# jinggqu/NextGen-UIA

Hardware: AMD Instinct MI355X
Metric: images/sec fwd+bwd BiomedCLIP+Mona bs=256 (higher is better)
Workload: dtype bf16

## Files before the change

### nextgen-uia_amd/csrc/mona.hip

```cpp
#include <stdlib.h>
#include <type_traits>
#include "uia_common.h"
#include "uia_kernels.h"

#include "mona_spatial.h"

namespace {
using namespace uia_mona;

constexpr int LN_MAXV = 4;

template <typename T>
__global__ __launch_bounds__(256) void mona_pre_fwd_kernel(int M, int D, const float* __restrict__ x, const float* __restrict__ nw,
                                                            const float* __restrict__ nb, const float* __restrict__ gamma,
                                                            const float* __restrict__ gammax, float eps, T* __restrict__ u) {
    const int row = blockIdx.x * 4 + (threadIdx.x >> 6), lane = threadIdx.x & 63;
    if (row >= M) return;
    const int nv = D >> 2;
    const float* xr = x + (size_t)row * D;
    f32x4 v[LN_MAXV];
    float s = 0.f;
#pragma unroll
    for (int k = 0; k < LN_MAXV; ++k) {
        const int c = lane + 64 * k;
// ... 514 lines not shown
        sdc = red[c * 50 + 49];
#pragma unroll
        for (int i = 0; i < 7; ++i)
#pragma unroll
            for (int j = 0; j < 7; ++j) {
                grad_out(wsrow, WS_C3W, p.g_conv3_w, c * 49 + i * 7 + j, w3 * dkm[i * 7 + j]);
                if (i >= 1 && i <= 5 && j >= 1 && j <= 5) grad_out(wsrow, WS_C2W, p.g_conv2_w, c * 25 + (i - 1) * 5 + (j - 1), w2 * dkm[i * 7 + j]);
                if (i >= 2 && i <= 4 && j >= 2 && j <= 4) grad_out(wsrow, WS_C1W, p.g_conv1_w, c * 9 + (i - 2) * 3 + (j - 2), w1 * dkm[i * 7 + j]);
            }
        grad_out(wsrow, WS_C1B, p.g_conv1_b, c, w1 * sdc);
        grad_out(wsrow, WS_C2B, p.g_conv2_b, c, w2 * sdc);
        grad_out(wsrow, WS_C3B, p.g_conv3_b, c, w3 * sdc);
    }
    float dpool_c = 0.f;
    if (has_noise) {
        __syncthreads();
        float r1 = wave_sum(dwm1), r2 = wave_sum(dwm2), r3 = wave_sum(dwm3);
        if (c == 0) { scr[SCR_RED + grp * 4] = r1; scr[SCR_RED + grp * 4 + 1] = r2; scr[SCR_RED + grp * 4 + 2] = r3; }
        __syncthreads();
        if (tid < 16) {
            float dwv[3], wv[3] = {w1, w2, w3}, dl[3];
            for (int k = 0; k < 3; ++k) {
                dwv[k] = 0.f;
                for (int q = 0; q < NGRP; ++q) dwv[k] += scr[SCR_RED + 4 * q + k];
            }
            const float dot = dwv[0] * wv[0] + dwv[1] * wv[1] + dwv[2] * wv[2];
            for (int k = 0; k < 3; ++k) dl[k] = wv[k] * (dwv[k] - dot);
            const float hid = scr[SCR_HID + tid], hpre = scr[SCR_HPRE + tid];
            float dh = 0.f;
            for (int k = 0; k < 3; ++k) {
                grad_out(wsrow, WS_NE3W, p.g_ne3_w, k * 16 + tid, dl[k] * hid);
                dh = fmaf(dl[k], p.ne3_w[k * 16 + tid], dh);
            }
            if (tid < 3) grad_out(wsrow, WS_NE3B, p.g_ne3_b, tid, dl[tid]);
            dh = hpre > 0.f ? dh : 0.f;
            scr[SCR_HPRE + tid] = dh;
            grad_out(wsrow, WS_NE1B, p.g_ne1_b, tid, dh);
        }
        __syncthreads();
        if (tid < 64) {
            float dp = 0.f;
            for (int j = 0; j < 16; ++j) dp = fmaf(scr[SCR_HPRE + j], p.ne1_w[j * 64 + tid], dp);
            scr[SCR_DPOOL + tid] = dp / hw;
        }
        for (int i = tid; i < 16 * 64; i += 512) grad_out(wsrow, WS_NE1W, p.g_ne1_w, i, scr[SCR_HPRE + (i >> 6)] * scr[SCR_POOL + (i & 63)]);
        __syncthreads();
        dpool_c = scr[SCR_DPOOL + c];
    }
    float dfc = 0.f;
    T* dt = (T*)p.dt;
    for (int px = p0; px < p1; ++px) {
        const int y = px / w, x = px - y * w;
        float acc = 0.f;
#pragma unroll
        for (int i = 0; i < 7; ++i) {
            const int yy = y - (i - 3);
            const bool vy = yy >= 0 && yy < h;
#pragma unroll
            for (int j = 0; j < 7; ++j) {
                const int xx = x - (j - 3);
                const bool ok = vy && xx >= 0 && xx < w;
                const float gv = gS[(ok ? 1 + yy * w + xx : 0) * BOTT + c];
                acc = fmaf(KM(i, j), ok ? gv : 0.f, acc);
            }
        }
        const float dxf = acc + dpool_c;
        dfc = fmaf(dxf, tS[(1 + px) * BOTT + c], dfc);
        dt[(tok0 + 1 + px) * BOTT + c] = from_f32<T>(fmaf(f, dxf, gS[(1 + px) * BOTT + c]));
    }
    if (grp == 0) dt[tok0 * BOTT + c] = from_f32<T>(gS[c]);
    if (has_freq) {
        __syncthreads();
        scr[SCR_PART + grp * 64 + c] = dfc;
        __syncthreads();
        if (tid < 64) {
            float a = 0.f;
#pragma unroll
            for (int q = 0; q < NGRP; ++q) a += scr[SCR_PART + q * 64 + tid];
            grad_out(wsrow, WS_FREQ, p.g_freq, tid, a);
        }
    }
}

template <int W, bool BWD>
__global__ __launch_bounds__(512) void mona_spatial_fast_kernel(const uia_mona_spatial_desc p) {
    typedef bf16_t T;
    extern __shared__ __attribute__((aligned(16))) char smem[];
    const int h = p.h, hw = h * W, ntok = hw + 1;
    float* tS = (float*)smem;
    float* cS = tS + ntok * BOTT;
    const int cs_floats = (hw * FLD > FAST_RED) ? hw * FLD : FAST_RED;
    float* gS = cS + cs_floats;
    float* scr = BWD ? gS + ((ntok * FLD > KW_FLOATS) ? ntok * FLD : KW_FLOATS) : cS + cs_floats;
    const int tid = threadIdx.x, lane = tid & 63, c = lane, grp = tid >> 6;
    const int li = lane & 15, g = lane >> 4;
    const int b = blockIdx.x;
    const bool has_freq = p.variant == UIA_MONA_FREQ_ENHANCED || p.variant == UIA_MONA_HYBRID;
    const bool has_noise = p.variant == UIA_MONA_NOISE_AWARE || p.variant == UIA_MONA_HYBRID;
    const int ppg = (hw + NGRP - 1) / NGRP;
    const size_t tok0 = (size_t)b * ntok;
    float* wsrow = (BWD && p.ws) ? p.ws + (size_t)b * WS_ROW : nullptr;

    float* wst = BWD ? gS : scr + SCR_SIZE;
    for (int i = tid; i < KW_FLOATS / 4; i += 512) {
        const float* src = i < 144 ? p.conv1_w + 4 * i : (i < 544 ? p.conv2_w + 4 * (i - 144) : p.conv3_w + 4 * (i - 544));
        *(f32x4*)(wst + 4 * i) = load4(src);
    }
    load_tokens((const T*)p.t + tok0 * BOTT, tS, ntok, tid);
    __syncthreads();
#if defined(MSB_STOP) && MSB_STOP == 0
    if (BWD && p.B > 0) return;
#endif
    const float f = has_freq ? p.freq[c] : 1.0f;
    float w1 = 1.f / 3.f, w2 = 1.f / 3.f, w3 = 1.f / 3.f;
    if (has_noise) {
        noise_forward(p, tS, f, hw, ppg, c, grp, tid, scr);
        w1 = scr[SCR_W]; w2 = scr[SCR_W + 1]; w3 = scr[SCR_W + 2];
    }
    float km[49];
    {
        float k1[9], k2[25], k3[49];
#pragma unroll
        for (int i = 0; i < 9; ++i) k1[i] = wst[c * 9 + i];
#pragma unroll
        for (int i = 0; i < 25; ++i) k2[i] = wst[576 + c * 25 + i];
#pragma unroll
        for (int i = 0; i < 49; ++i) k3[i] = wst[2176 + c * 49 + i];
#pragma unroll
        for (int i = 0; i < 7; ++i)
#pragma unroll
            for (int j = 0; j < 7; ++j) km[i * 7 + j] = KM(i, j);
    }
    const float b1 = p.conv1_b[c], b2 = p.conv2_b[c], b3 = p.conv3_b[c];
    const float bm = w1 * b1 + w2 * b2 + w3 * b3;
#if defined(MSB_STOP) && MSB_STOP == 1
    if (BWD && p.B > 0) return;
#endif
    for (int y = grp; y < h; y += NGRP) {
        float acc[W];
#pragma unroll
        for (int x = 0; x < W; ++x) acc[x] = 0.f;
        stencil_row<W, false>(tS + BOTT, BOTT, h, y, c, km, acc);
#pragma unroll
        for (int x = 0; x < W; ++x) cS[(y * W + x) * FLD + c] = fmaf(f, acc[x], bm) + tS[(1 + y * W + x) * BOTT + c];
    }
    __syncthreads();

#if defined(MSB_STOP) && MSB_STOP == 2
    if (BWD && p.B > 0) return;
#endif
    const float inv_keep = p.p_drop > 0.f ? 1.0f / (1.0f - p.p_drop) : 1.0f;
    const uint32_t thresh = p.p_drop > 0.f ? (uint32_t)fminf(p.p_drop * 4294967296.0f, 4294967295.0f) : 0u;
    auto keep_scale = [&](int tok, int ch) -> float {
        const size_t idx = (tok0 + tok) * BOTT + ch;
        if (p.keep_mask) return p.keep_mask[idx] ? inv_keep : 0.f;
        if (p.p_drop > 0.f) return dropout_keep(p.seed, (uint32_t)idx, thresh) ? inv_keep : 0.f;
        return 1.0f;
    };
    const int mtiles = (hw + 15) >> 4;
    {
        bf16x8 pw[4][2];
        float pb[4];
#pragma unroll
        for (int nt = 0; nt < 4; ++nt) {
#pragma unroll
            for (int kk = 0; kk < 2; ++kk) {
                const float* src = p.proj_w + (16 * nt + li) * 64 + 32 * kk + 8 * g;
                pw[nt][kk] = pack8(load4(src), load4(src + 4));
            }
            pb[nt] = p.proj_b[16 * nt + li];
        }
        for (int mt = grp; mt < mtiles; mt += NGRP) {
            int arow = 16 * mt + li;
            arow = arow < hw ? arow : hw - 1;
            bf16x8 af[2];
#pragma unroll
            for (int kk = 0; kk < 2; ++kk) {
                const float* src = cS + arow * FLD + 32 * kk + 8 * g;
                af[kk] = pack8(*(const f32x4*)src, *(const f32x4*)(src + 4));
            }
#pragma unroll
            for (int nt = 0; nt < 4; ++nt) {
                f32x4 acc = f32x4{0.f, 0.f, 0.f, 0.f};
                acc = __builtin_amdgcn_mfma_f32_16x16x32_bf16(af[0], pw[nt][0], acc, 0, 0, 0);
                acc = __builtin_amdgcn_mfma_f32_16x16x32_bf16(af[1], pw[nt][1], acc, 0, 0, 0);
                const int co = 16 * nt + li;
#pragma unroll
                for (int r = 0; r < 4; ++r) {
                    const int px = 16 * mt + 4 * g + r;
                    if (px < hw) {
                        const float z = cS[px * FLD + co] + acc[r] + pb[nt];
                        const float ks = keep_scale(1 + px, co);
                        if (!BWD) ((T*)p.d)[(tok0 + 1 + px) * BOTT + co] = (T)(gelu_erf(z) * ks);
                        else gS[(1 + px) * FLD + co] = to_f32(((const T*)p.dd)[(tok0 + 1 + px) * BOTT + co]) * ks * dgelu_erf(z);
                    }
                }
            }
        }
        if (grp == NGRP - 1) {
            const float z = tS[c], ks = keep_scale(0, c);
            if (!BWD) ((T*)p.d)[tok0 * BOTT + c] = (T)(gelu_erf(z) * ks);
            else gS[c] = to_f32(((const T*)p.dd)[tok0 * BOTT + c]) * ks * dgelu_erf(z);
        }
    }
    if (!BWD) return;

#if defined(MSB_STOP) && MSB_STOP == 3
    if (BWD && p.B > 0) return;
#endif
    __syncthreads();
    {
        const int mt = grp & 3, nt0 = 2 * (grp >> 2);
        f32x4 acc[2] = {f32x4{0.f, 0.f, 0.f, 0.f}, f32x4{0.f, 0.f, 0.f, 0.f}};
        const int ksteps = (hw + 31) >> 5;
        for (int ks = 0; ks < ksteps; ++ks) {
            bf16x8 a, al, bb[2], bl[2];
#pragma unroll
            for (int e = 0; e < 8; ++e) {
                const int px = 32 * ks + 8 * g + e;
                const int pc = px < hw ? px : hw - 1;
                const float av = px < hw ? gS[(1 + pc) * FLD + 16 * mt + li] : 0.f;
                const float b0 = cS[pc * FLD + 16 * nt0 + li], b1 = cS[pc * FLD + 16 * (nt0 + 1) + li];
                a[e] = (bf16_t)av;      al[e] = (bf16_t)(av - (float)a[e]);
                bb[0][e] = (bf16_t)b0;  bl[0][e] = (bf16_t)(b0 - (float)bb[0][e]);
                bb[1][e] = (bf16_t)b1;  bl[1][e] = (bf16_t)(b1 - (float)bb[1][e]);
            }
#pragma unroll
            for (int q = 0; q < 2; ++q) {
                acc[q] = __builtin_amdgcn_mfma_f32_16x16x32_bf16(al, bb[q], acc[q], 0, 0, 0);
                acc[q] = __builtin_amdgcn_mfma_f32_16x16x32_bf16(a, bl[q], acc[q], 0, 0, 0);
                acc[q] = __builtin_amdgcn_mfma_f32_16x16x32_bf16(a, bb[q], acc[q], 0, 0, 0);
            }
        }
#pragma unroll
        for (int q = 0; q < 2; ++q)
#pragma unroll
            for (int r = 0; r < 4; ++r) grad_out(wsrow, WS_PROJ_W, p.g_proj_w, (16 * mt + 4 * g + r) * 64 + 16 * (nt0 + q) + li, acc[q][r]);
        {
            float sb = 0.f;
            for (int px = grp; px < hw; px += NGRP) sb += gS[(1 + px) * FLD + c];
            scr[SCR_PART + grp * 64 + c] = sb;
        }
    }
    __syncthreads();
#if defined(MSB_STOP) && MSB_STOP == 4
    if (BWD && p.B > 0) return;
#endif
    {
        bf16x8 pt[4][2];
#pragma unroll
        for (int nt = 0; nt < 4; ++nt)
#pragma unroll
            for (int kk = 0; kk < 2; ++kk)
#pragma unroll
                for (int e = 0; e < 8; ++e) pt[nt][kk][e] = (bf16_t)p.proj_w[(32 * kk + 8 * g + e) * 64 + 16 * nt + li];
        for (int mt = grp; mt < mtiles; mt += NGRP) {
            int arow = 16 * mt + li;
            arow = arow < hw ? arow : hw - 1;
            bf16x8 af[2];
#pragma unroll
            for (int kk = 0; kk < 2; ++kk) {
                const float* src = gS + (1 + arow) * FLD + 32 * kk + 8 * g;
                af[kk] = pack8(*(const f32x4*)src, *(const f32x4*)(src + 4));
            }
            f32x4 acc[4];
#pragma unroll
            for (int nt = 0; nt < 4; ++nt) {
                acc[nt] = __builtin_amdgcn_mfma_f32_16x16x32_bf16(af[0], pt[nt][0], f32x4{0.f, 0.f, 0.f, 0.f}, 0, 0, 0);
                acc[nt] = __builtin_amdgcn_mfma_f32_16x16x32_bf16(af[1], pt[nt][1], acc[nt], 0, 0, 0);
            }
            __builtin_amdgcn_wave_barrier();
#pragma unroll
            for (int nt = 0; nt < 4; ++nt)
#pragma unroll
                for (int r = 0; r < 4; ++r) {
                    const int px = 16 * mt + 4 * g + r;
                    if (px < hw) gS[(1 + px) * FLD + 16 * nt + li] += acc[nt][r];
                }
        }
    }
    __syncthreads();
#if defined(MSB_STOP) && MSB_STOP == 5
    if (BWD && p.B > 0) return;
#endif
    float dkm[49];
#pragma unroll
    for (int i = 0; i < 49; ++i) dkm[i] = 0.f;
    float sdc = 0.f, dwm1 = 0.f, dwm2 = 0.f, dwm3 = 0.f;
    for (int y = grp; y < h; y += NGRP) {
        float dcr[W];
#pragma unroll
        for (int x = 0; x < W; ++x) { dcr[x] = gS[(1 + y * W + x) * FLD + c]; sdc += dcr[x]; }
#pragma unroll
        for (int i = 0; i < 7; ++i) {
            const int yy = y + i - 3;
            if (yy < 0 || yy >= h) continue;
            float row[W + 6];
#pragma unroll
            for (int x = 0; x < W + 6; ++x) row[x] = 0.f;
#pragma unroll
            for (int x = 0; x < W; ++x) row[3 + x] = tS[(1 + yy * W + x) * BOTT + c];
#pragma unroll
            for (int j = 0; j < 7; ++j) {
                float a = 0.f;
#pragma unroll
                for (int x = 0; x < W; ++x) a = fmaf(dcr[x], row[x + j], a);
                dkm[i * 7 + j] += a;
            }
        }
    }
    if (has_noise) {
        float s1 = 0.f, s2 = 0.f, s3 = 0.f;
#pragma unroll
        for (int i = 0; i < 7; ++i)
#pragma unroll
            for (int j = 0; j < 7; ++j) {
                s3 = fmaf(p.conv3_w[c * 49 + i * 7 + j], dkm[i * 7 + j], s3);
                if (i >= 1 && i <= 5 && j >= 1 && j <= 5) s2 = fmaf(p.conv2_w[c * 25 + (i - 1) * 5 + (j - 1)], dkm[i * 7 + j], s2);
                if (i >= 2 && i <= 4 && j >= 2 && j <= 4) s1 = fmaf(p.conv1_w[c * 9 + (i - 2) * 3 + (j - 2)], dkm[i * 7 + j], s1);
            }
        dwm1 = fmaf(f, s1, b1 * sdc);
        dwm2 = fmaf(f, s2, b2 * sdc);
        dwm3 = fmaf(f, s3, b3 * sdc);
    }
#if defined(MSB_STOP) && MSB_STOP == 6
    if (BWD && p.B > 0) return;
#endif
    float* red = cS;
    constexpr int RST = 51, RW = 64 * RST;
    if (grp >= 4) {
        float* dst = red + (grp - 4) * RW + c * RST;
#pragma unroll
        for (int i = 0; i < 49; ++i) dst[i] = dkm[i];
        dst[49] = sdc;
    }
    __syncthreads();
    if (grp < 4) {
        float* dst = red + grp * RW + c * RST;
#pragma unroll
        for (int i = 0; i < 49; ++i) dst[i] += dkm[i];
        dst[49] += sdc;
    }
    __syncthreads();
    auto red4 = [&](int ch, int k) { const float* r = red + ch * RST + k; return (r[0] + r[RW]) + (r[2 * RW] + r[3 * RW]); };
    for (int i = tid; i < 64 * 49; i += 512) {
        const int ch = i / 49, k = i - 49 * ch;
        grad_out(wsrow, WS_C3W, p.g_conv3_w, i, w3 * (has_freq ? p.freq[ch] : 1.0f) * red4(ch, k));
    }
    for (int i = tid; i < 64 * 25; i += 512) {
        const int ch = i / 25, k = i - 25 * ch, ki = k / 5, kj = k - 5 * ki;
        grad_out(wsrow, WS_C2W, p.g_conv2_w, i, w2 * (has_freq ? p.freq[ch] : 1.0f) * red4(ch, (ki + 1) * 7 + kj + 1));
    }
    for (int i = tid; i < 64 * 9; i += 512) {
        const int ch = i / 9, k = i - 9 * ch, ki = k / 3, kj = k - 3 * ki;
        grad_out(wsrow, WS_C1W, p.g_conv1_w, i, w1 * (has_freq ? p.freq[ch] : 1.0f) * red4(ch, (ki + 2) * 7 + kj + 2));
    }
    if (tid < 64) {
        const float sd = red4(tid, 49);
        grad_out(wsrow, WS_C1B, p.g_conv1_b, tid, w1 * sd);
        grad_out(wsrow, WS_C2B, p.g_conv2_b, tid, w2 * sd);
        grad_out(wsrow, WS_C3B, p.g_conv3_b, tid, w3 * sd);
    } else if (tid < 128) {
        float sb = 0.f;
#pragma unroll
        for (int q = 0; q < NGRP; ++q) sb += scr[SCR_PART + q * 64 + tid - 64];
        grad_out(wsrow, WS_PROJ_B, p.g_proj_b, tid - 64, sb);
    }
#if defined(MSB_STOP) && MSB_STOP == 7
    if (BWD && p.B > 0) return;
#endif
    float dpool_c = 0.f;
    if (has_noise) {
        __syncthreads();
        float r1 = wave_sum(dwm1), r2 = wave_sum(dwm2), r3 = wave_sum(dwm3);
        if (c == 0) { scr[SCR_RED + grp * 4] = r1; scr[SCR_RED + grp * 4 + 1] = r2; scr[SCR_RED + grp * 4 + 2] = r3; }
        __syncthreads();
        if (tid < 16) {
            float dwv[3], wv[3] = {w1, w2, w3}, dl[3];
            for (int k = 0; k < 3; ++k) {
                dwv[k] = 0.f;
                for (int q = 0; q < NGRP; ++q) dwv[k] += scr[SCR_RED + 4 * q + k];
            }
            const float dot = dwv[0] * wv[0] + dwv[1] * wv[1] + dwv[2] * wv[2];
            for (int k = 0; k < 3; ++k) dl[k] = wv[k] * (dwv[k] - dot);
            const float hid = scr[SCR_HID + tid], hpre = scr[SCR_HPRE + tid];
            float dh = 0.f;
            for (int k = 0; k < 3; ++k) {
                grad_out(wsrow, WS_NE3W, p.g_ne3_w, k * 16 + tid, dl[k] * hid);
                dh = fmaf(dl[k], p.ne3_w[k * 16 + tid], dh);
            }
            if (tid < 3) grad_out(wsrow, WS_NE3B, p.g_ne3_b, tid, dl[tid]);
            dh = hpre > 0.f ? dh : 0.f;
            scr[SCR_HPRE + tid] = dh;
            grad_out(wsrow, WS_NE1B, p.g_ne1_b, tid, dh);
        }
        __syncthreads();
        if (tid < 64) {
            float dp = 0.f;
            for (int j = 0; j < 16; ++j) dp = fmaf(scr[SCR_HPRE + j], p.ne1_w[j * 64 + tid], dp);
            scr[SCR_DPOOL + tid] = dp / hw;
        }
        for (int i = tid; i < 16 * 64; i += 512) grad_out(wsrow, WS_NE1W, p.g_ne1_w, i, scr[SCR_HPRE + (i >> 6)] * scr[SCR_POOL + (i & 63)]);
        __syncthreads();
        dpool_c = scr[SCR_DPOOL + c];
    }
#if defined(MSB_STOP) && MSB_STOP == 8
    if (BWD && p.B > 0) return;
#endif
    float dfc = 0.f;
    T* dt = (T*)p.dt;
    for (int y = grp; y < h; y += NGRP) {
        float acc[W];
#pragma unroll
        for (int x = 0; x < W; ++x) acc[x] = 0.f;
        stencil_row<W, true>(gS + FLD, FLD, h, y, c, km, acc);
#pragma unroll
        for (int x = 0; x < W; ++x) {
            const int px = y * W + x;
            const float dxf = acc[x] + dpool_c;
            dfc = fmaf(dxf, tS[(1 + px) * BOTT + c], dfc);
            dt[(tok0 + 1 + px) * BOTT + c] = (T)fmaf(f, dxf, gS[(1 + px) * FLD + c]);
        }
    }
    if (grp == NGRP - 1) dt[tok0 * BOTT + c] = (T)gS[c];
#if defined(MSB_STOP) && MSB_STOP == 9
    if (BWD && p.B > 0) return;
#endif
    if (has_freq) {
        __syncthreads();
        scr[SCR_PART + grp * 64 + c] = dfc;
        __syncthreads();
        if (tid < 64) {
            float a = 0.f;
#pragma unroll
            for (int q = 0; q < NGRP; ++q) a += scr[SCR_PART + q * 64 + tid];
            grad_out(wsrow, WS_FREQ, p.g_freq, tid, a);
        }
    }
}

constexpr int WSR_PH = 16;
__global__ __launch_bounds__(64 * WSR_PH) void mona_ws_reduce_kernel(int B, const float* __restrict__ ws, uia_mona_spatial_desc p, int has_freq, int has_noise) {
    __shared__ float part[WSR_PH][64];
    const int cx = threadIdx.x & 63, ph = threadIdx.x >> 6;
    const int col = blockIdx.x * 64 + cx;
    float s = 0.f;
    if (col < WS_ROW) {
        float a[4] = {0.f, 0.f, 0.f, 0.f};
        int b = ph;
        for (; b + 3 * WSR_PH < B; b += 4 * WSR_PH) {
#pragma unroll
            for (int k = 0; k < 4; ++k) a[k] += ws[(size_t)(b + WSR_PH * k) * WS_ROW + col];
        }
        for (; b < B; b += WSR_PH) a[0] += ws[(size_t)b * WS_ROW + col];
        s = (a[0] + a[1]) + (a[2] + a[3]);
    }
    part[ph][cx] = s;
    __syncthreads();
    if (ph != 0 || col >= WS_ROW) return;
    s = 0.f;
#pragma unroll
    for (int q = 0; q < WSR_PH; q += 4) s += (part[q][cx] + part[q + 1][cx]) + (part[q + 2][cx] + part[q + 3][cx]);
    float* dst = nullptr;
    int idx = 0;
    if (col < WS_PROJ_B) { dst = p.g_proj_w; idx = col - WS_PROJ_W; }
    else if (col < WS_C1W) { dst = p.g_proj_b; idx = col - WS_PROJ_B; }
    else if (col < WS_C1B) { dst = p.g_conv1_w; idx = col - WS_C1W; }
    else if (col < WS_C2W) { dst = p.g_conv1_b; idx = col - WS_C1B; }
    else if (col < WS_C2B) { dst = p.g_conv2_w; idx = col - WS_C2W; }
    else if (col < WS_C3W) { dst = p.g_conv2_b; idx = col - WS_C2B; }
    else if (col < WS_C3B) { dst = p.g_conv3_w; idx = col - WS_C3W; }
    else if (col < WS_FREQ) { dst = p.g_conv3_b; idx = col - WS_C3B; }
    else if (col < WS_NE1W) { if (!has_freq) return; dst = p.g_freq; idx = col - WS_FREQ; }
    else if (!has_noise) return;
    else if (col < WS_NE1B) { dst = p.g_ne1_w; idx = col - WS_NE1W; }
    else if (col < WS_NE3W) { dst = p.g_ne1_b; idx = col - WS_NE1B; }
    else if (col < WS_NE3B) { dst = p.g_ne3_w; idx = col - WS_NE3W; if (idx >= 48) return; }
    else { dst = p.g_ne3_b; idx = col - WS_NE3B; if (idx >= 3) return; }
    atomicAdd(dst + idx, s);
}

size_t spatial_lds(int hw, bool bwd) {
    const size_t tile = (size_t)(hw + 1) * BOTT;
    const size_t cs = bwd ? (tile > (size_t)RED_FLOATS ? tile : (size_t)RED_FLOATS) : tile;
    return (tile * (bwd ? 2 : 1) + cs + SCR_SIZE) * sizeof(float);
}

template <int W, bool BWD>
int launch_spatial_fast(hipStream_t stream, const uia_mona_spatial_desc& p) {
    auto kern = mona_spatial_fast_kernel<W, BWD>;
    static UiaDevOnce attr_once;
    UIA_ENSURE_LDS_ATTR(attr_once, kern, 160 * 1024);
    hipLaunchKernelGGL(kern, dim3(p.B), dim3(512), spatial_fast_lds(p.h * W, BWD), stream, p);
    return 0;
}

template <typename T, bool BWD>
int launch_spatial(hipStream_t stream, const uia_mona_spatial_desc& p) {
    const size_t lds = spatial_lds(p.h * p.w, BWD);
    bool fast = false;
    if (sizeof(T) == 2 && (p.w == 14 || p.w == 4) && spatial_fast_lds(p.h * p.w, BWD) <= 160 * 1024) {
        static int allow = -1;
        if (allow < 0) { const char* e = getenv("UIA_MONA_FAST"); allow = (e && e[0] == '0') ? 0 : 1; }
        fast = allow != 0;
    }
    if (fast) {
        if (p.w == 14) launch_spatial_fast<14, BWD>(stream, p);
        else launch_spatial_fast<4, BWD>(stream, p);
    } else {
    auto kern = mona_spatial_kernel<T, BWD>;
    static UiaDevOnce attr_once;
    UIA_ENSURE_LDS_ATTR(attr_once, kern, 160 * 1024);
    hipLaunchKernelGGL(kern, dim3(p.B), dim3(512), lds, stream, p);
    }
    if (BWD && p.ws) {
        const bool has_freq = p.variant == UIA_MONA_FREQ_ENHANCED || p.variant == UIA_MONA_HYBRID;
        const bool has_noise = p.variant == UIA_MONA_NOISE_AWARE || p.variant == UIA_MONA_HYBRID;
        const int cols = has_noise ? WS_ROW : (has_freq ? WS_NE1W : WS_FREQ);
        hipLaunchKernelGGL(mona_ws_reduce_kernel, dim3((cols + 63) / 64), dim3(64 * WSR_PH), 0, stream, p.B, p.ws, p, (int)has_freq, (int)has_noise);
    }
    UIA_CHECK_LAUNCH();
    return 0;
}

int check_spatial(const uia_mona_spatial_desc& p, bool bwd) {
    UIA_CHECK_ARG(p.variant >= 0 && p.variant <= 3, "uia_mona_spatial: bad variant %d", p.variant);
    UIA_CHECK_ARG(p.bott == BOTT, "uia_mona_spatial: bottleneck %d unsupported (64 only)", p.bott);
    UIA_CHECK_ARG(p.B > 0 && p.h > 0 && p.w > 0, "uia_mona_spatial: empty problem");
    UIA_CHECK_ARG(spatial_lds(p.h * p.w, bwd) <= 160 * 1024, "uia_mona_spatial: %dx%d grid does not fit the 160 KiB LDS tile", p.h, p.w);
    UIA_CHECK_ARG(p.t && p.conv1_w && p.conv1_b && p.conv2_w && p.conv2_b && p.conv3_w && p.conv3_b && p.proj_w && p.proj_b, "uia_mona_spatial: null parameter");
    const bool has_freq = p.variant == UIA_MONA_FREQ_ENHANCED || p.variant == UIA_MONA_HYBRID;
    const bool has_noise = p.variant == UIA_MONA_NOISE_AWARE || p.variant == UIA_MONA_HYBRID;
    UIA_CHECK_ARG(!has_freq || p.freq, "uia_mona_spatial: variant needs freq_filter");
    UIA_CHECK_ARG(!has_noise || (p.ne1_w && p.ne1_b && p.ne3_w && p.ne3_b), "uia_mona_spatial: variant needs noise_estimator parameters");
    UIA_CHECK_ARG(p.p_drop >= 0.f && p.p_drop < 1.f, "uia_mona_spatial: p_drop %f", p.p_drop);
    UIA_CHECK_ARG((((uintptr_t)p.conv1_w | (uintptr_t)p.conv2_w | (uintptr_t)p.conv3_w | (uintptr_t)p.proj_w) & 15) == 0,
                  "uia_mona_spatial: conv / projector weights must be 16-byte aligned");
    if (!bwd) { UIA_CHECK_ARG(p.d, "uia_mona_spatial_fwd: null output"); }
    else {
        UIA_CHECK_ARG(p.dd && p.dt && p.g_conv1_w && p.g_conv1_b && p.g_conv2_w && p.g_conv2_b && p.g_conv3_w && p.g_conv3_b && p.g_proj_w && p.g_proj_b,
                      "uia_mona_spatial_bwd: null gradient buffer");
        UIA_CHECK_ARG(!has_freq || p.g_freq, "uia_mona_spatial_bwd: variant needs g_freq");
        UIA_CHECK_ARG(!has_noise || (p.g_ne1_w && p.g_ne1_b && p.g_ne3_w && p.g_ne3_b), "uia_mona_spatial_bwd: variant needs noise_estimator gradient buffers");
    }
    return 0;
}

}

int uia_mona_pre_fwd_t_launch(hipStream_t stream, int dtype, int M, int D, const float* x, const float* nw, const float* nb, const float* gamma,
                              const float* gammax, float eps, void* u, const void* w1, long ldw1, const float* b1, void* t, long ldt) {
    UIA_CHECK_ARG(dtype == UIA_BF16 && D == 768 && M > 0, "uia_mona_pre_fwd_t: bf16, D = 768 (got dtype %d, D = %d)", dtype, D);
    UIA_CHECK_ARG(x && nw && nb && gamma && gammax && u && w1 && t && ldw1 >= D && ldw1 % 8 == 0 && ldt >= 64 && ldt % 4 == 0 && (uintptr_t)w1 % 16 == 0 && (uintptr_t)t % 8 == 0 &&
                      (!b1 || (uintptr_t)b1 % 16 == 0),
                  "uia_mona_pre_fwd_t: null tensor, or W1 [64, D] / t [M, 64] rows not 16- / 8-byte aligned");
    constexpr int KS = 24;
    const int lds = 16 * (2 * 32 * KS + 16);
    const int ntiles = (M + 15) / 16;
    int blocks = ntiles;
    int per_cu = 0, dev = 0, ncu = 0;
    if (hipOccupancyMaxActiveBlocksPerMultiprocessor(&per_cu, mona_pre_fwd_t_kernel<KS>, 256, lds) == hipSuccess && per_cu > 0 && hipGetDevice(&dev) == hipSuccess &&
        hipDeviceGetAttribute(&ncu, hipDeviceAttributeMultiprocessorCount, dev) == hipSuccess && ncu > 0 && per_cu * ncu < blocks) blocks = per_cu * ncu;
    hipLaunchKernelGGL(mona_pre_fwd_t_kernel<KS>, dim3(blocks), dim3(256), lds, stream, M, x, nw, nb, gamma, gammax, eps, (bf16_t*)u, (const bf16_t*)w1, ldw1, b1, (bf16_t*)t, ldt);
    UIA_CHECK_LAUNCH();
    return 0;
}

int uia_mona_pre_fwd_launch(hipStream_t stream, int dtype, int M, int D, const float* x, const float* nw, const float* nb, const float* gamma,
                            const float* gammax, float eps, void* u) {
    UIA_CHECK_ARG(M > 0 && D > 0 && D % 4 == 0 && D <= 1024, "uia_mona_pre_fwd: unsupported shape M=%d D=%d", M, D);
    UIA_CHECK_ARG(x && nw && nb && gamma && gammax && u, "uia_mona_pre_fwd: null tensor");
    const dim3 grid((M + 3) / 4), block(256);
    if (dtype == UIA_BF16) hipLaunchKernelGGL(mona_pre_fwd_kernel<bf16_t>, grid, block, 0, stream, M, D, x, nw, nb, gamma, gammax, eps, (bf16_t*)u);
    else if (dtype == UIA_F32) hipLaunchKernelGGL(mona_pre_fwd_kernel<float>, grid, block, 0, stream, M, D, x, nw, nb, gamma, gammax, eps, (float*)u);
    else { uia_set_error("uia_mona_pre_fwd: bad dtype %d", dtype); return -1; }
    UIA_CHECK_LAUNCH();
// ... 82 lines not shown
```

### nextgen-uia_amd/csrc/mona_spatial.h

```cpp
#pragma once
#include "uia_common.h"
#include "uia_kernels.h"

namespace uia_mona {

constexpr int BOTT = 64;

#define KM(i, j) (w3 * k3[(i) * 7 + (j)] + (((i) >= 1 && (i) <= 5 && (j) >= 1 && (j) <= 5) ? w2 * k2[((i) - 1) * 5 + ((j) - 1)] : 0.f) + \
                  (((i) >= 2 && (i) <= 4 && (j) >= 2 && (j) <= 4) ? w1 * k1[((i) - 2) * 3 + ((j) - 2)] : 0.f))

template <typename T>
__device__ __forceinline__ void load_tokens(const T* __restrict__ src, float* __restrict__ dst, int ntok, int tid) {
    for (int i = tid; i < ntok * 8; i += 512) {
        float v[8];
        load8(src + (size_t)i * 8, v);
#pragma unroll
        for (int e = 0; e < 8; ++e) dst[i * 8 + e] = v[e];
    }
}

constexpr int NGRP = 8;
constexpr int SCR_PART = 0, SCR_POOL = 512, SCR_HPRE = 576, SCR_HID = 592, SCR_W = 608, SCR_DPOOL = 616, SCR_RED = 680, SCR_SIZE = 720;
constexpr int RED_FLOATS = 64 * 50;
constexpr int WS_PROJ_W = 0, WS_PROJ_B = 4096, WS_C1W = 4160, WS_C1B = 4736, WS_C2W = 4800, WS_C2B = 6400, WS_C3W = 6464, WS_C3B = 9600,
              WS_FREQ = 9664, WS_NE1W = 9728, WS_NE1B = 10752, WS_NE3W = 10768, WS_NE3B = 10816, WS_ROW = 10880;

__device__ __forceinline__ void noise_forward(const uia_mona_spatial_desc& p, const float* tS, float f, int hw, int ppg, int c, int grp,
                                              int tid, float* scr) {
    float s = 0.f;
    const int p0 = grp * ppg, p1 = min(hw, p0 + ppg);
    for (int px = p0; px < p1; ++px) s += tS[(1 + px) * BOTT + c];
    scr[SCR_PART + grp * 64 + c] = s;
    __syncthreads();
    if (tid < 64) {
        float a = 0.f;
#pragma unroll
        for (int q = 0; q < NGRP; ++q) a += scr[SCR_PART + q * 64 + tid];
        scr[SCR_POOL + tid] = f * a / hw;
    }
    __syncthreads();
    if (tid < 16) {
        float a = p.ne1_b[tid];
        for (int k = 0; k < 64; ++k) a = fmaf(p.ne1_w[tid * 64 + k], scr[SCR_POOL + k], a);
        scr[SCR_HPRE + tid] = a;
        scr[SCR_HID + tid] = fmaxf(a, 0.f);
    }
    __syncthreads();
    if (tid == 0) {
        float l[3];
        for (int k = 0; k < 3; ++k) {
            float a = p.ne3_b[k];
            for (int j = 0; j < 16; ++j) a = fmaf(p.ne3_w[k * 16 + j], scr[SCR_HID + j], a);
            l[k] = a;
        }
        const float m = fmaxf(l[0], fmaxf(l[1], l[2]));
        const float e0 = expf(l[0] - m), e1 = expf(l[1] - m), e2 = expf(l[2] - m), inv = 1.f / (e0 + e1 + e2);
        scr[SCR_W + 0] = e0 * inv; scr[SCR_W + 1] = e1 * inv; scr[SCR_W + 2] = e2 * inv;
    }
    __syncthreads();
}

constexpr int FLD = 68;
constexpr int FAST_RED = 4 * 64 * 51;
constexpr int KW_FLOATS = 64 * (9 + 25 + 49);
__host__ __device__ constexpr size_t spatial_fast_lds(int hw, bool bwd) {
    return ((size_t)(hw + 1) * BOTT + (size_t)((hw * FLD > FAST_RED) ? hw * FLD : FAST_RED) +
            (bwd ? (size_t)(((hw + 1) * FLD > KW_FLOATS) ? (hw + 1) * FLD : KW_FLOATS) : (size_t)KW_FLOATS) + SCR_SIZE) * sizeof(float);
}
__device__ __forceinline__ bf16x8 pack8(const f32x4& a, const f32x4& b) {
    bf16x8 r = {(bf16_t)a[0], (bf16_t)a[1], (bf16_t)a[2], (bf16_t)a[3], (bf16_t)b[0], (bf16_t)b[1], (bf16_t)b[2], (bf16_t)b[3]};
    return r;
}

template <int W, bool FLIP>
__device__ __forceinline__ void stencil_row(const float* __restrict__ src, int ld, int h, int y, int c, const float (&km)[49], float (&acc)[W]) {
#pragma unroll
    for (int i = 0; i < 7; ++i) {
        const int yy = FLIP ? y - (i - 3) : y + (i - 3);
        if (yy < 0 || yy >= h) continue;
        float row[W + 6];
#pragma unroll
        for (int x = 0; x < W + 6; ++x) row[x] = 0.f;
#pragma unroll
        for (int x = 0; x < W; ++x) row[3 + x] = src[(size_t)(yy * W + x) * ld + c];
#pragma unroll
        for (int x = 0; x < W; ++x)
#pragma unroll
            for (int j = 0; j < 7; ++j) acc[x] = fmaf(km[i * 7 + j], row[3 + x + (FLIP ? -(j - 3) : (j - 3))], acc[x]);
    }
}


}
```

Measured before the change: 6804.

## Widen Mona spatial kernel to 1024 threads with packed-FMA stencil and staged I/O

Raises the fused Mona spatial kernel from 8 to 16 waves per block and redistributes the work: each wave now handles one 16-column output tile of the projection, one 16x16 tile of the projection weight gradient, and one kernel-row share of the depthwise-conv weight gradient. The 7x7 stencil switches to v_pk_fma_f32 inline asm, computing two output pixels per instruction. Projection outputs and incoming gradients are staged through LDS so global bf16 traffic uses 8-wide vector loads and stores. The noise-branch reduction is restructured to run in one wave. The changes add register pressure and inline asm and rely on the LDS reduction region being large enough.

```diff
diff --git a/nextgen-uia_amd/csrc/mona.hip b/nextgen-uia_amd/csrc/mona.hip
--- a/nextgen-uia_amd/csrc/mona.hip
+++ b/nextgen-uia_amd/csrc/mona.hip
@@ -620,8 +620,40 @@
     }
 }
 
+typedef float f32x2 __attribute__((ext_vector_type(2)));
+__device__ __forceinline__ void pk_fma_tap(f32x2& acc, const f32x2& kk, int half, const f32x2& r) {
+    if (half == 0) asm("v_pk_fma_f32 %0, %1, %2, %0 op_sel_hi:[0,1,1]" : "+v"(acc) : "v"(kk), "v"(r));
+    else asm("v_pk_fma_f32 %0, %1, %2, %0 op_sel:[1,0,0] op_sel_hi:[1,1,1]" : "+v"(acc) : "v"(kk), "v"(r));
+}
+template <int W, bool FLIP>
+__device__ __forceinline__ void stencil_row_pk(const float* __restrict__ src, int ld, int h, int y, int c, const f32x2 (&km2)[25], f32x2 (&acc)[W / 2]) {
+    static_assert(W % 2 == 0, "pairs of outputs");
+#pragma unroll
+    for (int i = 0; i < 7; ++i) {
+        const int yy = FLIP ? y - (i - 3) : y + (i - 3);
+        if (yy < 0 || yy >= h) continue;
+        float row[W + 6];
+#pragma unroll
+        for (int x = 0; x < W + 6; ++x) row[x] = 0.f;
+#pragma unroll
+        for (int x = 0; x < W; ++x) row[3 + x] = src[(size_t)(yy * W + x) * ld + c];
+        f32x2 re[(W + 6) / 2], ro[(W + 4) / 2];
+#pragma unroll
+        for (int k = 0; k < (W + 6) / 2; ++k) re[k] = f32x2{row[2 * k], row[2 * k + 1]};
+#pragma unroll
+        for (int k = 0; k < (W + 4) / 2; ++k) ro[k] = f32x2{row[2 * k + 1], row[2 * k + 2]};
+#pragma unroll
+        for (int xp = 0; xp < W / 2; ++xp)
+#pragma unroll
+            for (int j = 0; j < 7; ++j) {
+                const int t = i * 7 + j, s = 3 + 2 * xp + (FLIP ? -(j - 3) : (j - 3));
+                pk_fma_tap(acc[xp], km2[t >> 1], t & 1, (s & 1) ? ro[(s - 1) >> 1] : re[s >> 1]);
+            }
+    }
+}
+
 template <int W, bool BWD>
-__global__ __launch_bounds__(512) void mona_spatial_fast_kernel(const uia_mona_spatial_desc p) {
+__global__ __launch_bounds__(FTHR) void mona_spatial_fast_kernel(const uia_mona_spatial_desc p) {
     typedef bf16_t T;
     extern __shared__ __attribute__((aligned(16))) char smem[];
     const int h = p.h, hw = h * W, ntok = hw + 1;
@@ -640,11 +672,11 @@
     float* wsrow = (BWD && p.ws) ? p.ws + (size_t)b * WS_ROW : nullptr;
 
     float* wst = BWD ? gS : scr + SCR_SIZE;
-    for (int i = tid; i < KW_FLOATS / 4; i += 512) {
+    for (int i = tid; i < KW_FLOATS / 4; i += FTHR) {
         const float* src = i < 144 ? p.conv1_w + 4 * i : (i < 544 ? p.conv2_w + 4 * (i - 144) : p.conv3_w + 4 * (i - 544));
         *(f32x4*)(wst + 4 * i) = load4(src);
     }
-    load_tokens((const T*)p.t + tok0 * BOTT, tS, ntok, tid);
+    load_tokens((const T*)p.t + tok0 * BOTT, tS, ntok, tid, FTHR);
     __syncthreads();
 #if defined(MSB_STOP) && MSB_STOP == 0
     if (BWD && p.B > 0) return;
@@ -655,32 +687,28 @@
         noise_forward(p, tS, f, hw, ppg, c, grp, tid, scr);
         w1 = scr[SCR_W]; w2 = scr[SCR_W + 1]; w3 = scr[SCR_W + 2];
     }
-    float km[49];
-    {
-        float k1[9], k2[25], k3[49];
-#pragma unroll
-        for (int i = 0; i < 9; ++i) k1[i] = wst[c * 9 + i];
-#pragma unroll
-        for (int i = 0; i < 25; ++i) k2[i] = wst[576 + c * 25 + i];
-#pragma unroll
-        for (int i = 0; i < 49; ++i) k3[i] = wst[2176 + c * 49 + i];
+    f32x2 km2[25];
+    auto merge_taps = [&](const float* img) {
+        const float *k1 = img + c * 9, *k2 = img + 576 + c * 25, *k3 = img + 2176 + c * 49;
 #pragma unroll
         for (int i = 0; i < 7; ++i)
 #pragma unroll
-            for (int j = 0; j < 7; ++j) km[i * 7 + j] = KM(i, j);
-    }
+            for (int j = 0; j < 7; ++j) km2[(i * 7 + j) >> 1][(i * 7 + j) & 1] = KM(i, j);
+        km2[24][1] = 0.f;
+    };
+    merge_taps(wst);
     const float b1 = p.conv1_b[c], b2 = p.conv2_b[c], b3 = p.conv3_b[c];
     const float bm = w1 * b1 + w2 * b2 + w3 * b3;
 #if defined(MSB_STOP) && MSB_STOP == 1
     if (BWD && p.B > 0) return;
 #endif
-    for (int y = grp; y < h; y += NGRP) {
-        float acc[W];
-#pragma unroll
-        for (int x = 0; x < W; ++x) acc[x] = 0.f;
-        stencil_row<W, false>(tS + BOTT, BOTT, h, y, c, km, acc);
-#pragma unroll
-        for (int x = 0; x < W; ++x) cS[(y * W + x) * FLD + c] = fmaf(f, acc[x], bm) + tS[(1 + y * W + x) * BOTT + c];
+    for (int y = grp; y < h; y += FGRP) {
+        f32x2 acc[W / 2];
+#pragma unroll
+        for (int x = 0; x < W / 2; ++x) acc[x] = f32x2{0.f, 0.f};
+        stencil_row_pk<W, false>(tS + BOTT, BOTT, h, y, c, km2, acc);
+#pragma unroll
+        for (int x = 0; x < W; ++x) cS[(y * W + x) * FLD + c] = fmaf(f, acc[x >> 1][x & 1], bm) + tS[(1 + y * W + x) * BOTT + c];
     }
     __syncthreads();
 
@@ -697,18 +725,28 @@
     };
     const int mtiles = (hw + 15) >> 4;
     {
-        bf16x8 pw[4][2];
-        float pb[4];
-#pragma unroll
-        for (int nt = 0; nt < 4; ++nt) {
-#pragma unroll
-            for (int kk = 0; kk < 2; ++kk) {
-                const float* src = p.proj_w + (16 * nt + li) * 64 + 32 * kk + 8 * g;
-                pw[nt][kk] = pack8(load4(src), load4(src + 4));
-            }
-            pb[nt] = p.proj_b[16 * nt + li];
-        }
-        for (int mt = grp; mt < mtiles; mt += NGRP) {
+        const int nt = grp & 3, co = 16 * nt + li;
+        bf16x8 pw[2];
+#pragma unroll
+        for (int kk = 0; kk < 2; ++kk) {
+            const float* src = p.proj_w + co * 64 + 32 * kk + 8 * g;
+            pw[kk] = pack8(load4(src), load4(src + 4));
+        }
+        const float pb = p.proj_b[co];
+        const int prow = lane >> 1, pcol = 16 * nt + 8 * (lane & 1);
+        const bool wide = ((uintptr_t)(BWD ? p.dd : p.d) & 15) == 0;
+        for (int mt = grp >> 2; mt < mtiles; mt += FGRP / 4) {
+            const int ppx = 16 * mt + prow;
+            if (BWD && lane < 32 && ppx < hw) {
+                const T* src = (const T*)p.dd + (tok0 + 1 + ppx) * BOTT + pcol;
+                float v[8];
+                if (wide) load8(src, v);
+                else {
+#pragma unroll
+                    for (int e = 0; e < 8; ++e) v[e] = to_f32(src[e]);
+                }
+                store8(gS + (1 + ppx) * FLD + pcol, v);
+            }
             int arow = 16 * mt + li;
             arow = arow < hw ? arow : hw - 1;
             bf16x8 af[2];
@@ -717,25 +755,41 @@
                 const float* src = cS + arow * FLD + 32 * kk + 8 * g;
                 af[kk] = pack8(*(const f32x4*)src, *(const f32x4*)(src + 4));
             }
-#pragma unroll
-            for (int nt = 0; nt < 4; ++nt) {
-                f32x4 acc = f32x4{0.f, 0.f, 0.f, 0.f};
-                acc = __builtin_amdgcn_mfma_f32_16x16x32_bf16(af[0], pw[nt][0], acc, 0, 0, 0);
-                acc = __builtin_amdgcn_mfma_f32_16x16x32_bf16(af[1], pw[nt][1], acc, 0, 0, 0);
-                const int co = 16 * nt + li;
-#pragma unroll
-                for (int r = 0; r < 4; ++r) {
-                    const int px = 16 * mt + 4 * g + r;
-                    if (px < hw) {
-                        const float z = cS[px * FLD + co] + acc[r] + pb[nt];
-                        const float ks = keep_scale(1 + px, co);
-                        if (!BWD) ((T*)p.d)[(tok0 + 1 + px) * BOTT + co] = (T)(gelu_erf(z) * ks);
-                        else gS[(1 + px) * FLD + co] = to_f32(((const T*)p.dd)[(tok0 + 1 + px) * BOTT + co]) * ks * dgelu_erf(z);
+            __builtin_amdgcn_fence(__ATOMIC_ACQ_REL, "wavefront");
+            __builtin_amdgcn_wave_barrier();
+            f32x4 acc = f32x4{0.f, 0.f, 0.f, 0.f};
+            acc = __builtin_amdgcn_mfma_f32_16x16x32_bf16(af[0], pw[0], acc, 0, 0, 0);
+            acc = __builtin_amdgcn_mfma_f32_16x16x32_bf16(af[1], pw[1], acc, 0, 0, 0);
+#pragma unroll
+            for (int r = 0; r < 4; ++r) {
+                const int px = 16 * mt + 4 * g + r, pc = px < hw ? px : hw - 1;
+                const float z = cS[pc * FLD + co] + acc[r] + pb;
+                const float ks = keep_scale(1 + pc, co);
+                if (!BWD) {
+                    const float v = gelu_erf(z) * ks;
+                    if (px < hw) tS[(1 + px) * BOTT + co] = v;
+                } else {
+                    float* q = gS + (1 + pc) * FLD + co;
+                    const float v = *q * ks * dgelu_erf(z);
+                    if (px < hw) *q = v;
+                }
+            }
+            if (!BWD) {
+                __builtin_amdgcn_fence(__ATOMIC_ACQ_REL, "wavefront");
+                __builtin_amdgcn_wave_barrier();
+                if (lane < 32 && ppx < hw) {
+                    float v[8];
+                    load8(tS + (1 + ppx) * BOTT + pcol, v);
+                    T* dst = (T*)p.d + (tok0 + 1 + ppx) * BOTT + pcol;
+                    if (wide) store8(dst, v);
+                    else {
+#pragma unroll
+                        for (int e = 0; e < 8; ++e) dst[e] = (T)v[e];
                     }
                 }
             }
         }
-        if (grp == NGRP - 1) {
+        if (grp == FGRP - 1) {
             const float z = tS[c], ks = keep_scale(0, c);
             if (!BWD) ((T*)p.d)[tok0 * BOTT + c] = (T)(gelu_erf(z) * ks);
             else gS[c] = to_f32(((const T*)p.dd)[tok0 * BOTT + c]) * ks * dgelu_erf(z);
@@ -748,33 +802,29 @@
 #endif
     __syncthreads();
     {
-        const int mt = grp & 3, nt0 = 2 * (grp >> 2);
-        f32x4 acc[2] = {f32x4{0.f, 0.f, 0.f, 0.f}, f32x4{0.f, 0.f, 0.f, 0.f}};
         const int ksteps = (hw + 31) >> 5;
+        for (int tile = grp; tile < 16; tile += FGRP) {
+        const int mt = tile & 3, nt = tile >> 2;
+        f32x4 acc = f32x4{0.f, 0.f, 0.f, 0.f};
         for (int ks = 0; ks < ksteps; ++ks) {
-            bf16x8 a, al, bb[2], bl[2];
+            bf16x8 a, al, bb, bl;
 #pragma unroll
             for (int e = 0; e < 8; ++e) {
                 const int px = 32 * ks + 8 * g + e;
                 const int pc = px < hw ? px : hw - 1;
                 const float av = px < hw ? gS[(1 + pc) * FLD + 16 * mt + li] : 0.f;
-                const float b0 = cS[pc * FLD + 16 * nt0 + li], b1 = cS[pc * FLD + 16 * (nt0 + 1) + li];
-                a[e] = (bf16_t)av;      al[e] = (bf16_t)(av - (float)a[e]);
-                bb[0][e] = (bf16_t)b0;  bl[0][e] = (bf16_t)(b0 - (float)bb[0][e]);
-                bb[1][e] = (bf16_t)b1;  bl[1][e] = (bf16_t)(b1 - (float)bb[1][e]);
-            }
-#pragma unroll
-            for (int q = 0; q < 2; ++q) {
-                acc[q] = __builtin_amdgcn_mfma_f32_16x16x32_bf16(al, bb[q], acc[q], 0, 0, 0);
-                acc[q] = __builtin_amdgcn_mfma_f32_16x16x32_bf16(a, bl[q], acc[q], 0, 0, 0);
-                acc[q] = __builtin_amdgcn_mfma_f32_16x16x32_bf16(a, bb[q], acc[q], 0, 0, 0);
-            }
-        }
-#pragma unroll
-        for (int q = 0; q < 2; ++q)
-#pragma unroll
-            for (int r = 0; r < 4; ++r) grad_out(wsrow, WS_PROJ_W, p.g_proj_w, (16 * mt + 4 * g + r) * 64 + 16 * (nt0 + q) + li, acc[q][r]);
-        {
+                const float bv = cS[pc * FLD + 16 * nt + li];
+                a[e] = (bf16_t)av;   al[e] = (bf16_t)(av - (float)a[e]);
+                bb[e] = (bf16_t)bv;  bl[e] = (bf16_t)(bv - (float)bb[e]);
+            }
+            acc = __builtin_amdgcn_mfma_f32_16x16x32_bf16(al, bb, acc, 0, 0, 0);
+            acc = __builtin_amdgcn_mfma_f32_16x16x32_bf16(a, bl, acc, 0, 0, 0);
+            acc = __builtin_amdgcn_mfma_f32_16x16x32_bf16(a, bb, acc, 0, 0, 0);
+        }
+#pragma unroll
+        for (int r = 0; r < 4; ++r) grad_out(wsrow, WS_PROJ_W, p.g_proj_w, (16 * mt + 4 * g + r) * 64 + 16 * nt + li, acc[r]);
+        }
+        if (grp < NGRP) {
             float sb = 0.f;
             for (int px = grp; px < hw; px += NGRP) sb += gS[(1 + px) * FLD + c];
             scr[SCR_PART + grp * 64 + c] = sb;
@@ -792,7 +842,7 @@
             for (int kk = 0; kk < 2; ++kk)
 #pragma unroll
                 for (int e = 0; e < 8; ++e) pt[nt][kk][e] = (bf16_t)p.proj_w[(32 * kk + 8 * g + e) * 64 + 16 * nt + li];
-        for (int mt = grp; mt < mtiles; mt += NGRP) {
+        for (int mt = grp; mt < mtiles; mt += FGRP) {
             int arow = 16 * mt + li;
             arow = arow < hw ? arow : hw - 1;
             bf16x8 af[2];
@@ -821,19 +871,31 @@
 #if defined(MSB_STOP) && MSB_STOP == 5
     if (BWD && p.B > 0) return;
 #endif
-    float dkm[49];
-#pragma unroll
-    for (int i = 0; i < 49; ++i) dkm[i] = 0.f;
-    float sdc = 0.f, dwm1 = 0.f, dwm2 = 0.f, dwm3 = 0.f;
-    for (int y = grp; y < h; y += NGRP) {
-        float dcr[W];
-#pragma unroll
-        for (int x = 0; x < W; ++x) { dcr[x] = gS[(1 + y * W + x) * FLD + c]; sdc += dcr[x]; }
-#pragma unroll
-        for (int i = 0; i < 7; ++i) {
+    float* red = cS;
+    constexpr int RST = 51, RW = 64 * RST;
+    float* wst2 = red + 2 * RW;
+    static_assert(FGRP == 8 || FGRP == 16, "pass A deals 7 tap rows x FGRP / 8 row shares");
+    static_assert(2 * RW + KW_FLOATS <= FAST_RED, "the second weight image lies behind the reduction images");
+    constexpr int NWI = (KW_FLOATS / 4 + FTHR - 1) / FTHR;
+    f32x4 wimg[NWI];
+#pragma unroll
+    for (int q = 0; q < NWI; ++q) {
+        const int i = tid + q * FTHR;
+        const float* src = i < 144 ? p.conv1_w + 4 * i : (i < 544 ? p.conv2_w + 4 * (i - 144) : p.conv3_w + 4 * (i - 544));
+        if (i < KW_FLOATS / 4) wimg[q] = load4(src);
+    }
+    constexpr int NH = FGRP / 8;
+    if (grp < 7 * NH) {
+        const int i = grp % 7, half = grp / 7;
+        float dk7[7];
+#pragma unroll
+        for (int j = 0; j < 7; ++j) dk7[j] = 0.f;
+        for (int y = half; y < h; y += NH) {
             const int yy = y + i - 3;
             if (yy < 0 || yy >= h) continue;
-            float row[W + 6];
+            float dcr[W], row[W + 6];
+#pragma unroll
+            for (int x = 0; x < W; ++x) dcr[x] = gS[(1 + y * W + x) * FLD + c];
 #pragma unroll
             for (int x = 0; x < W + 6; ++x) row[x] = 0.f;
 #pragma unroll
@@ -843,94 +905,87 @@
                 float a = 0.f;
 #pragma unroll
                 for (int x = 0; x < W; ++x) a = fmaf(dcr[x], row[x + j], a);
-                dkm[i * 7 + j] += a;
-            }
-        }
-    }
-    if (has_noise) {
-        float s1 = 0.f, s2 = 0.f, s3 = 0.f;
-#pragma unroll
-        for (int i = 0; i < 7; ++i)
-#pragma unroll
-            for (int j = 0; j < 7; ++j) {
-                s3 = fmaf(p.conv3_w[c * 49 + i * 7 + j], dkm[i * 7 + j], s3);
-                if (i >= 1 && i <= 5 && j >= 1 && j <= 5) s2 = fmaf(p.conv2_w[c * 25 + (i - 1) * 5 + (j - 1)], dkm[i * 7 + j], s2);
-                if (i >= 2 && i <= 4 && j >= 2 && j <= 4) s1 = fmaf(p.conv1_w[c * 9 + (i - 2) * 3 + (j - 2)], dkm[i * 7 + j], s1);
-            }
-        dwm1 = fmaf(f, s1, b1 * sdc);
-        dwm2 = fmaf(f, s2, b2 * sdc);
-        dwm3 = fmaf(f, s3, b3 * sdc);
+                dk7[j] += a;
+            }
+        }
+        float* dst = red + half * RW + c * RST + i * 7;
+#pragma unroll
+        for (int j = 0; j < 7; ++j) dst[j] = dk7[j];
+    } else {
+        const int half = grp - 7 * NH;
+        float sdc = 0.f;
+        for (int y = half; y < h; y += NH)
+#pragma unroll
+            for (int x = 0; x < W; ++x) sdc += gS[(1 + y * W + x) * FLD + c];
+        red[half * RW + c * RST + 49] = sdc;
+    }
+#pragma unroll
+    for (int q = 0; q < NWI; ++q) {
+        const int i = tid + q * FTHR;
+        if (i < KW_FLOATS / 4) *(f32x4*)(wst2 + 4 * i) = wimg[q];
     }
 #if defined(MSB_STOP) && MSB_STOP == 6
     if (BWD && p.B > 0) return;
 #endif
-    float* red = cS;
-    constexpr int RST = 51, RW = 64 * RST;
-    if (grp >= 4) {
-        float* dst = red + (grp - 4) * RW + c * RST;
-#pragma unroll
-        for (int i = 0; i < 49; ++i) dst[i] = dkm[i];
-        dst[49] = sdc;
-    }
-    __syncthreads();
-    if (grp < 4) {
-        float* dst = red + grp * RW + c * RST;
-#pragma unroll
-        for (int i = 0; i < 49; ++i) dst[i] += dkm[i];
-        dst[49] += sdc;
-    }
-    __syncthreads();
-    auto red4 = [&](int ch, int k) { const float* r = red + ch * RST + k; return (r[0] + r[RW]) + (r[2 * RW] + r[3 * RW]); };
-    for (int i = tid; i < 64 * 49; i += 512) {
+    __syncthreads();
+    auto red2 = [&](int ch, int k) { const float* r = red + ch * RST + k; return NH == 2 ? r[0] + r[RW] : r[0]; };
+    for (int i = tid; i < 64 * 49; i += FTHR) {
         const int ch = i / 49, k = i - 49 * ch;
-        grad_out(wsrow, WS_C3W, p.g_conv3_w, i, w3 * (has_freq ? p.freq[ch] : 1.0f) * red4(ch, k));
-    }
-    for (int i = tid; i < 64 * 25; i += 512) {
+        grad_out(wsrow, WS_C3W, p.g_conv3_w, i, w3 * (has_freq ? p.freq[ch] : 1.0f) * red2(ch, k));
+    }
+    for (int i = tid; i < 64 * 25; i += FTHR) {
         const int ch = i / 25, k = i - 25 * ch, ki = k / 5, kj = k - 5 * ki;
-        grad_out(wsrow, WS_C2W, p.g_conv2_w, i, w2 * (has_freq ? p.freq[ch] : 1.0f) * red4(ch, (ki + 1) * 7 + kj + 1));
-    }
-    for (int i = tid; i < 64 * 9; i += 512) {
+        grad_out(wsrow, WS_C2W, p.g_conv2_w, i, w2 * (has_freq ? p.freq[ch] : 1.0f) * red2(ch, (ki + 1) * 7 + kj + 1));
+    }
+    for (int i = tid; i < 64 * 9; i += FTHR) {
         const int ch = i / 9, k = i - 9 * ch, ki = k / 3, kj = k - 3 * ki;
-        grad_out(wsrow, WS_C1W, p.g_conv1_w, i, w1 * (has_freq ? p.freq[ch] : 1.0f) * red4(ch, (ki + 2) * 7 + kj + 2));
-    }
-    if (tid < 64) {
-        const float sd = red4(tid, 49);
-        grad_out(wsrow, WS_C1B, p.g_conv1_b, tid, w1 * sd);
-        grad_out(wsrow, WS_C2B, p.g_conv2_b, tid, w2 * sd);
-        grad_out(wsrow, WS_C3B, p.g_conv3_b, tid, w3 * sd);
-    } else if (tid < 128) {
+        grad_out(wsrow, WS_C1W, p.g_conv1_w, i, w1 * (has_freq ? p.freq[ch] : 1.0f) * red2(ch, (ki + 2) * 7 + kj + 2));
+    }
+    if (grp == FGRP - 1) {
+        const float sd = red2(c, 49);
+        grad_out(wsrow, WS_C1B, p.g_conv1_b, c, w1 * sd);
+        grad_out(wsrow, WS_C2B, p.g_conv2_b, c, w2 * sd);
+        grad_out(wsrow, WS_C3B, p.g_conv3_b, c, w3 * sd);
+    } else if (grp == FGRP - 2) {
         float sb = 0.f;
 #pragma unroll
-        for (int q = 0; q < NGRP; ++q) sb += scr[SCR_PART + q * 64 + tid - 64];
-        grad_out(wsrow, WS_PROJ_B, p.g_proj_b, tid - 64, sb);
+        for (int q = 0; q < NGRP; ++q) sb += scr[SCR_PART + q * 64 + c];
+        grad_out(wsrow, WS_PROJ_B, p.g_proj_b, c, sb);
     }
 #if defined(MSB_STOP) && MSB_STOP == 7
     if (BWD && p.B > 0) return;
 #endif
     float dpool_c = 0.f;
     if (has_noise) {
-        __syncthreads();
-        float r1 = wave_sum(dwm1), r2 = wave_sum(dwm2), r3 = wave_sum(dwm3);
-        if (c == 0) { scr[SCR_RED + grp * 4] = r1; scr[SCR_RED + grp * 4 + 1] = r2; scr[SCR_RED + grp * 4 + 2] = r3; }
-        __syncthreads();
-        if (tid < 16) {
-            float dwv[3], wv[3] = {w1, w2, w3}, dl[3];
-            for (int k = 0; k < 3; ++k) {
-                dwv[k] = 0.f;
-                for (int q = 0; q < NGRP; ++q) dwv[k] += scr[SCR_RED + 4 * q + k];
-            }
-            const float dot = dwv[0] * wv[0] + dwv[1] * wv[1] + dwv[2] * wv[2];
-            for (int k = 0; k < 3; ++k) dl[k] = wv[k] * (dwv[k] - dot);
-            const float hid = scr[SCR_HID + tid], hpre = scr[SCR_HPRE + tid];
-            float dh = 0.f;
-            for (int k = 0; k < 3; ++k) {
-                grad_out(wsrow, WS_NE3W, p.g_ne3_w, k * 16 + tid, dl[k] * hid);
-                dh = fmaf(dl[k], p.ne3_w[k * 16 + tid], dh);
-            }
-            if (tid < 3) grad_out(wsrow, WS_NE3B, p.g_ne3_b, tid, dl[tid]);
-            dh = hpre > 0.f ? dh : 0.f;
-            scr[SCR_HPRE + tid] = dh;
-            grad_out(wsrow, WS_NE1B, p.g_ne1_b, tid, dh);
+        if (grp == 0) {
+            float s1 = 0.f, s2 = 0.f, s3 = 0.f;
+#pragma unroll
+            for (int i = 0; i < 7; ++i)
+#pragma unroll
+                for (int j = 0; j < 7; ++j) {
+                    const float dk = red2(c, i * 7 + j);
+                    s3 = fmaf(p.conv3_w[c * 49 + i * 7 + j], dk, s3);
+                    if (i >= 1 && i <= 5 && j >= 1 && j <= 5) s2 = fmaf(p.conv2_w[c * 25 + (i - 1) * 5 + (j - 1)], dk, s2);
+                    if (i >= 2 && i <= 4 && j >= 2 && j <= 4) s1 = fmaf(p.conv1_w[c * 9 + (i - 2) * 3 + (j - 2)], dk, s1);
+                }
+            const float sdc = red2(c, 49);
+            const float r1 = wave_sum(fmaf(f, s1, b1 * sdc)), r2 = wave_sum(fmaf(f, s2, b2 * sdc)), r3 = wave_sum(fmaf(f, s3, b3 * sdc));
+            if (tid < 16) {
+                const float dwv[3] = {r1, r2, r3}, wv[3] = {w1, w2, w3};
+                float dl[3];
+                const float dot = dwv[0] * wv[0] + dwv[1] * wv[1] + dwv[2] * wv[2];
+                for (int k = 0; k < 3; ++k) dl[k] = wv[k] * (dwv[k] - dot);
+                const float hid = scr[SCR_HID + tid], hpre = scr[SCR_HPRE + tid];
+                float dh = 0.f;
+                for (int k = 0; k < 3; ++k) {
+                    grad_out(wsrow, WS_NE3W, p.g_ne3_w, k * 16 + tid, dl[k] * hid);
+                    dh = fmaf(dl[k], p.ne3_w[k * 16 + tid], dh);
+                }
+                if (tid < 3) grad_out(wsrow, WS_NE3B, p.g_ne3_b, tid, dl[tid]);
+                dh = hpre > 0.f ? dh : 0.f;
+                scr[SCR_HPRE + tid] = dh;
+                grad_out(wsrow, WS_NE1B, p.g_ne1_b, tid, dh);
+            }
         }
         __syncthreads();
         if (tid < 64) {
@@ -938,7 +993,7 @@
             for (int j = 0; j < 16; ++j) dp = fmaf(scr[SCR_HPRE + j], p.ne1_w[j * 64 + tid], dp);
             scr[SCR_DPOOL + tid] = dp / hw;
         }
-        for (int i = tid; i < 16 * 64; i += 512) grad_out(wsrow, WS_NE1W, p.g_ne1_w, i, scr[SCR_HPRE + (i >> 6)] * scr[SCR_POOL + (i & 63)]);
+        for (int i = tid; i < 16 * 64; i += FTHR) grad_out(wsrow, WS_NE1W, p.g_ne1_w, i, scr[SCR_HPRE + (i >> 6)] * scr[SCR_POOL + (i & 63)]);
         __syncthreads();
         dpool_c = scr[SCR_DPOOL + c];
     }
@@ -947,31 +1002,32 @@
 #endif
     float dfc = 0.f;
     T* dt = (T*)p.dt;
-    for (int y = grp; y < h; y += NGRP) {
-        float acc[W];
-#pragma unroll
-        for (int x = 0; x < W; ++x) acc[x] = 0.f;
-        stencil_row<W, true>(gS + FLD, FLD, h, y, c, km, acc);
+    merge_taps(wst2);
+    for (int y = grp; y < h; y += FGRP) {
+        f32x2 acc[W / 2];
+#pragma unroll
+        for (int x = 0; x < W / 2; ++x) acc[x] = f32x2{0.f, 0.f};
+        stencil_row_pk<W, true>(gS + FLD, FLD, h, y, c, km2, acc);
 #pragma unroll
         for (int x = 0; x < W; ++x) {
             const int px = y * W + x;
-            const float dxf = acc[x] + dpool_c;
+            const float dxf = acc[x >> 1][x & 1] + dpool_c;
             dfc = fmaf(dxf, tS[(1 + px) * BOTT + c], dfc);
             dt[(tok0 + 1 + px) * BOTT + c] = (T)fmaf(f, dxf, gS[(1 + px) * FLD + c]);
         }
     }
-    if (grp == NGRP - 1) dt[tok0 * BOTT + c] = (T)gS[c];
+    if (grp == FGRP - 1) dt[tok0 * BOTT + c] = (T)gS[c];
 #if defined(MSB_STOP) && MSB_STOP == 9
     if (BWD && p.B > 0) return;
 #endif
     if (has_freq) {
         __syncthreads();
-        scr[SCR_PART + grp * 64 + c] = dfc;
+        red[grp * 64 + c] = dfc;
         __syncthreads();
         if (tid < 64) {
             float a = 0.f;
 #pragma unroll
-            for (int q = 0; q < NGRP; ++q) a += scr[SCR_PART + q * 64 + tid];
+            for (int q = 0; q < FGRP; ++q) a += red[q * 64 + tid];
             grad_out(wsrow, WS_FREQ, p.g_freq, tid, a);
         }
     }
@@ -1029,7 +1085,7 @@
     auto kern = mona_spatial_fast_kernel<W, BWD>;
     static UiaDevOnce attr_once;
     UIA_ENSURE_LDS_ATTR(attr_once, kern, 160 * 1024);
-    hipLaunchKernelGGL(kern, dim3(p.B), dim3(512), spatial_fast_lds(p.h * W, BWD), stream, p);
+    hipLaunchKernelGGL(kern, dim3(p.B), dim3(FTHR), spatial_fast_lds(p.h * W, BWD), stream, p);
     return 0;
 }
 
diff --git a/nextgen-uia_amd/csrc/mona_spatial.h b/nextgen-uia_amd/csrc/mona_spatial.h
--- a/nextgen-uia_amd/csrc/mona_spatial.h
+++ b/nextgen-uia_amd/csrc/mona_spatial.h
@@ -10,8 +10,8 @@
                   (((i) >= 2 && (i) <= 4 && (j) >= 2 && (j) <= 4) ? w1 * k1[((i) - 2) * 3 + ((j) - 2)] : 0.f))
 
 template <typename T>
-__device__ __forceinline__ void load_tokens(const T* __restrict__ src, float* __restrict__ dst, int ntok, int tid) {
-    for (int i = tid; i < ntok * 8; i += 512) {
+__device__ __forceinline__ void load_tokens(const T* __restrict__ src, float* __restrict__ dst, int ntok, int tid, int nthr = 512) {
+    for (int i = tid; i < ntok * 8; i += nthr) {
         float v[8];
         load8(src + (size_t)i * 8, v);
 #pragma unroll
@@ -27,10 +27,12 @@
 
 __device__ __forceinline__ void noise_forward(const uia_mona_spatial_desc& p, const float* tS, float f, int hw, int ppg, int c, int grp,
                                               int tid, float* scr) {
-    float s = 0.f;
-    const int p0 = grp * ppg, p1 = min(hw, p0 + ppg);
-    for (int px = p0; px < p1; ++px) s += tS[(1 + px) * BOTT + c];
-    scr[SCR_PART + grp * 64 + c] = s;
+    if (grp < NGRP) {
+        float s = 0.f;
+        const int p0 = grp * ppg, p1 = min(hw, p0 + ppg);
+        for (int px = p0; px < p1; ++px) s += tS[(1 + px) * BOTT + c];
+        scr[SCR_PART + grp * 64 + c] = s;
+    }
     __syncthreads();
     if (tid < 64) {
         float a = 0.f;
@@ -61,6 +63,7 @@
 }
 
 constexpr int FLD = 68;
+constexpr int FGRP = 16, FTHR = 64 * FGRP;
 constexpr int FAST_RED = 4 * 64 * 51;
 constexpr int KW_FLOATS = 64 * (9 + 25 + 49);
 __host__ __device__ constexpr size_t spatial_fast_lds(int hw, bool bwd) {
```

Result: no change. 6828 (median of 6 runs) (+0.3%).
